# JuanDuGit/DH3D

Hardware: AMD Instinct MI355X
Metric: point-clouds/sec (higher is better)
Workload: dtype f32; 1 GPU; local-descriptor forward (basic_config), N=8192 K=8, batch=8; clouds_per_gpu=8, clouds_total=8, points=8192, knn=8, parallelism=clouds sharded over 1 GPU(s), no data-path collective, weights=random-init (no checkpoint blobs exist upstream), steps_in_flight=4

## Files before the change

dh3d_amd/csrc/knn.hip:

```cpp
#include <float.h>
#include <limits.h>

#include <type_traits>

#include "cell_walk.h"
#include "common.h"
#include "group_box.h"
#include "keys.h"
#include "wave_ops.h"

#pragma clang fp contract(off)

namespace {

typedef float f32x2 __attribute__((ext_vector_type(2)));
typedef unsigned long long u64;

constexpr int kQueriesPerBlock = 256;
constexpr int kChunk = 1024;
constexpr int kQueue = 16;

struct KnnLadder {
  int log2ct;
  int ctmask;
// ... 548 lines not shown
#pragma unroll
  for (int c = 0; c < CPL; ++c) kd[c] = ln + 64 * c < N ? __float_as_uint(sqrtf(s[c])) : 0xFFFFFFFFu;
  u64 need = 0;
  u64 m1 = ~0ull, m2 = ~0ull;
  bool more = false;
  auto rescan = [&]() {
    m1 = ~0ull; m2 = ~0ull;
    int cnt = 0;
    asm volatile("" : "+v"(ln));
#pragma unroll
    for (int c = 0; c < CPL; ++c) {
      const int j = ln + 64 * c;
      const unsigned tb = j < N ? (unsigned)((j & lad.ctmask) * lad.cv + (j >> lad.log2ct)) : 0xFFFFFFFFu;
      const u64 key = ((u64)kd[c] << 32) | tb;
      const bool ok = key >= need && key != ~0ull;
      const bool c1 = ok && key < m1, c2 = ok && key < m2;
      m2 = c1 ? m1 : (c2 ? key : m2);
      m1 = c1 ? key : m1;
      cnt += ok ? 1 : 0;
    }
    more = cnt > 2;
  };
  rescan();
  for (int r = 0; r < K; ++r) {
    const unsigned hi = wave_min_u32((unsigned)(m1 >> 32));
    const unsigned lo = wave_min_u32((unsigned)(m1 >> 32) == hi ? (unsigned)m1 : 0xFFFFFFFFu);
    if (lane == r) { my_hi = hi; my_lo = lo; }
    const u64 sel = ((u64)hi << 32) | lo;
    if (sel == ~0ull) break;
    need = sel + 1;
    const bool won = m1 == sel;
    const bool dry = won && m2 == ~0ull && more;
    m1 = won ? m2 : m1;
    m2 = won ? ~0ull : m2;
    if (__ballot(dry) != 0ull) rescan();
  }
}

template <int CPL, bool XYZ>
__global__ __launch_bounds__(256) void knn_small_kernel(const float *__restrict__ pos, int N, int K, KnnLadder lad,
                                                       int32_t *__restrict__ nn, float *__restrict__ dist, int Q) {
  __shared__ uint2 s_strip[4][64];
  const int b = blockIdx.y, lane = threadIdx.x & 63;
  const int wave = __builtin_amdgcn_readfirstlane(threadIdx.x >> 6);
  const int q0 = (blockIdx.x * 4 + wave) * Q;
  if (q0 >= N) return;
  const float *base = pos + (size_t)b * N * 3;
  float cx[CPL], cy[CPL], cz[CPL];
#pragma unroll
  for (int c = 0; c < CPL; ++c) {
    const int j = lane + 64 * c, jj = j < N ? j : 0;
    const float x = XYZ ? base[(size_t)jj * 3] : base[jj];
    cx[c] = j < N ? x : __builtin_nanf("");
    cy[c] = XYZ ? base[(size_t)jj * 3 + 1] : base[(size_t)N + jj];
    cz[c] = XYZ ? base[(size_t)jj * 3 + 2] : base[(size_t)2 * N + jj];
  }
  uint2 *strip = s_strip[wave];
#pragma unroll 1
  for (int qi = 0; qi < Q; ++qi) {
    const int q = q0 + qi;
    if (q >= N) break;
    const float qx = XYZ ? base[(size_t)q * 3] : base[q];
    const float qy = XYZ ? base[(size_t)q * 3 + 1] : base[(size_t)N + q];
    const float qz = XYZ ? base[(size_t)q * 3 + 2] : base[(size_t)2 * N + q];
    float s[CPL];
    float smin = __builtin_inff();
#pragma unroll
    for (int c = 0; c < CPL; ++c) {
      const float dx = qx - cx[c], dy = qy - cy[c], dz = qz - cz[c];
      s[c] = __builtin_fmaf(dz, dz, __builtin_fmaf(dy, dy, dx * dx));
      smin = fminf(smin, s[c]);
    }
    unsigned my_hi = 0xFFFFFFFFu, my_lo = 0xFFFFFFFFu;
    bool screened = K <= 8;
    int cnt = 0;
    if (screened) {
      const float ub = __fmul_rn(wave_max_of_min8_f32(smin), 1.000001f);
      int ln = lane;
      asm volatile("" : "+v"(ln));
#pragma unroll
      for (int c = 0; c < CPL; ++c) {
        const bool in = s[c] <= ub;
        const u64 mk = __ballot(in);
        const int at0 = cnt;
        cnt += __popcll(mk);
        if (in && cnt <= 64) {
          const unsigned at = __builtin_amdgcn_mbcnt_hi((unsigned)(mk >> 32), __builtin_amdgcn_mbcnt_lo((unsigned)mk, 0u));
          (strip + at0)[at] = make_uint2(__float_as_uint(s[c]), (unsigned)(ln + 64 * c));
        }
      }
      screened = cnt <= 64 && (cnt >= K || cnt >= N);
    }
    if (screened) {
      __builtin_amdgcn_fence(__ATOMIC_RELEASE, "wavefront");
      __builtin_amdgcn_wave_barrier();
      __builtin_amdgcn_fence(__ATOMIC_ACQUIRE, "wavefront");
      const uint2 e = strip[lane];
      const float d = sqrtf(__uint_as_float(e.x));
      const int j = (int)e.y;
      unsigned khi = lane < cnt ? __float_as_uint(d) : 0xFFFFFFFFu;
      unsigned klo = lane < cnt ? (unsigned)((j & lad.ctmask) * lad.cv + (j >> lad.log2ct)) : 0xFFFFFFFFu;
      for (int r = 0; r < K; ++r) {
        const unsigned hi = wave_min_u32(khi);
        const unsigned lo = wave_min_u32(khi == hi ? klo : 0xFFFFFFFFu);
        if (lane == r) { my_hi = hi; my_lo = lo; }
        if ((hi & lo) == 0xFFFFFFFFu) break;
        const bool won = khi == hi && klo == lo;
        khi = won ? 0xFFFFFFFFu : khi;
        klo = won ? 0xFFFFFFFFu : klo;
      }
      __builtin_amdgcn_fence(__ATOMIC_RELEASE, "wavefront");
    } else {
      knn_small_select_all<CPL>(s, N, K, lad, lane, my_hi, my_lo);
    }
    if (lane < K) {
      const size_t o = ((size_t)b * N + q) * K + lane;
      knn_emit(((u64)my_hi << 32) | my_lo, lad, nn + o, dist + o);
    }
  }
}

constexpr int kKnnMaxK = 64, kKnnMaxB = 65535;

static int knn_list_width(int K) { return K <= 4 ? 4 : K <= 8 ? 8 : K <= 16 ? 16 : K <= 32 ? 32 : 64; }

struct KnnPlan {
  int cpl, q, kmax;
};
static KnnPlan knn_plan(int B, int N, int K) {
  KnnPlan p{0, 0, 0};
  if (N <= 2048) {
    p.cpl = N <= 512 ? 8 : N <= 1024 ? 16 : 32;
    p.q = (long long)B * N <= 16384 ? 2 : 4;
    return p;
  }
  p.kmax = knn_list_width(K);
  return p;
}

constexpr int kAnyDpMax = 16;
static int knn_anydp_width(int K) { return K <= 8 ? 8 : K <= 16 ? 16 : 64; }

template <bool XYZ>
int knn_launch(const float *pos, int B, int N, int K, int32_t *nn, float *dist, hipStream_t s) {
  const KnnLadder lad = knn_ladder(N);
  const KnnPlan p = knn_plan(B, N, K);
  if (p.cpl > 0) {
    dim3 sgrid(dh3d_cdiv(N, 4 * p.q), B), sblock(256);
#define DH3D_SMALL_CASE(CPL)                                                                                     \
  if (p.cpl == CPL) {                                                                                            \
    hipLaunchKernelGGL((knn_small_kernel<CPL, XYZ>), sgrid, sblock, 0, s, pos, N, K, lad, nn, dist, p.q);        \
    return dh3d_launch_status();                                                                                 \
  }
    DH3D_SMALL_CASE(8) DH3D_SMALL_CASE(16) DH3D_SMALL_CASE(32)
#undef DH3D_SMALL_CASE
    return DH3D_ERR_UNSUPPORTED;
  }
  dim3 grid(dh3d_cdiv(N, kQueriesPerBlock), B), block(kQueriesPerBlock);
#define DH3D_LANE_CASE(KM)                                                                                       \
  if (p.kmax == KM) {                                                                                            \
    hipLaunchKernelGGL((knn_kernel<KM, XYZ>), grid, block, 0, s, pos, N, K, lad, nn, dist);                      \
    return dh3d_launch_status();                                                                                 \
  }
  DH3D_LANE_CASE(4) DH3D_LANE_CASE(8) DH3D_LANE_CASE(16) DH3D_LANE_CASE(32) DH3D_LANE_CASE(64)
#undef DH3D_LANE_CASE
  return DH3D_ERR_UNSUPPORTED;
}

template <int KMAX>
__global__ __launch_bounds__(256) void knn_anydp_kernel(const float *__restrict__ pos, int Dp, int N, int K, KnnLadder lad,
                                                        int32_t *__restrict__ nn, float *__restrict__ dist) {
  __shared__ float s_c[16][256];
  const int b = blockIdx.y, y = blockIdx.x * 256 + threadIdx.x;
  const float *pc = pos + (size_t)b * Dp * N;
  float q[16];
#pragma unroll
  for (int dp = 0; dp < 16; ++dp) q[dp] = (dp < Dp && y < N) ? pc[(size_t)dp * N + y] : 0.f;
  u64 keys[KMAX];
#pragma unroll
  for (int i = 0; i < KMAX; ++i) keys[i] = kKnnNoKey;
  for (int x0 = 0; x0 < N; x0 += 256) {
    __syncthreads();
    for (int dp = 0; dp < Dp; ++dp) s_c[dp][threadIdx.x] = x0 + (int)threadIdx.x < N ? pc[(size_t)dp * N + x0 + threadIdx.x] : 0.f;
    __syncthreads();
    const int cnt = min(256, N - x0);
    for (int j = 0; j < cnt; ++j) {
      float sum = 0.f;
      for (int dp = 0; dp < Dp; ++dp) {
        const float val = s_c[dp][j] - q[dp];
        sum = __builtin_fmaf(val, val, sum);
      }
      const float d = sqrtf(sum);
      const int x = x0 + j;
      const unsigned tb = (unsigned)((x & lad.ctmask) * lad.cv + (x >> lad.log2ct));
      const u64 key = ((u64)__float_as_uint(d) << 32) | tb;
      if (key < keys[K - 1]) {
        int i = K - 1;
        while (i > 0 && keys[i - 1] > key) { keys[i] = keys[i - 1]; --i; }
        keys[i] = key;
      }
    }
  }
  if (y >= N) return;
  int32_t *o_nn = nn + ((size_t)b * N + y) * K;
  float *o_d = dist + ((size_t)b * N + y) * K;
  for (int i = 0; i < K; ++i) knn_emit(keys[i], lad, o_nn + i, o_d + i);
}

}

DH3D_API int dh3d_knn_bruteforce(const float *positions, int B, int Dp, int N, int K, int32_t *nn,
                                 float *dist, void *stream) {
  DH3D_REQUIRE(positions && nn && dist && B > 0 && N > 0 && K > 0 && Dp > 0);
  DH3D_SUPPORTED(K <= kKnnMaxK && B <= kKnnMaxB);
  if (Dp == 3) return knn_launch<false>(positions, B, N, K, nn, dist, (hipStream_t)stream);
  DH3D_SUPPORTED(Dp <= kAnyDpMax);
  const KnnLadder lad = knn_ladder(N);
  dim3 grid(dh3d_cdiv(N, 256), B), block(256);
  hipStream_t s = (hipStream_t)stream;
  const int km = knn_anydp_width(K);
#define DH3D_ANYDP_CASE(KM)                                                                                      \
  if (km == KM) {                                                                                                \
    hipLaunchKernelGGL(knn_anydp_kernel<KM>, grid, block, 0, s, positions, Dp, N, K, lad, nn, dist);             \
    return dh3d_launch_status();                                                                                 \
  }
  DH3D_ANYDP_CASE(8) DH3D_ANYDP_CASE(16) DH3D_ANYDP_CASE(64)
#undef DH3D_ANYDP_CASE
  return DH3D_ERR_UNSUPPORTED;
}

DH3D_API int dh3d_knn_bruteforce_xyz(const float *xyz, int B, int N, int K, int32_t *nn, float *dist,
                                     void *stream) {
  DH3D_REQUIRE(xyz && nn && dist && B > 0 && N > 0 && K > 0);
  DH3D_SUPPORTED(K <= kKnnMaxK && B <= kKnnMaxB);
  return knn_launch<true>(xyz, B, N, K, nn, dist, (hipStream_t)stream);
}

DH3D_API int dh3d_knn_bruteforce_plan(int B, int Dp, int N, int K) {
  if (!(B > 0 && N > 0 && K > 0 && Dp > 0) || !(K <= kKnnMaxK && B <= kKnnMaxB)) return -1;
  if (Dp != 3) return Dp <= kAnyDpMax ? 3 * 65536 + knn_anydp_width(K) : -1;
  const KnnPlan p = knn_plan(B, N, K);
  return p.cpl > 0 ? 1 * 65536 + p.cpl * 256 + p.q : 2 * 65536 + p.kmax;
}

struct KnnSortedPlan {
  int s, kmax;
};
static KnnSortedPlan knn_sorted_plan(int B, int N, int K) {
  const long long groups = (long long)((N + 63) / 64) * B;
  KnnSortedPlan p{groups <= 256 ? 8 : groups <= 1280 ? 4 : groups <= 4096 ? 2 : 0, knn_list_width(K)};
  if (p.kmax > 16) p.s = 0;
  if (p.s == 8 && p.kmax == 4) p.kmax = 8;
  return p;
}

static int knn_sorted_launch(const float *sorted, const float *gbox, int B, int N, int K, int32_t *nn, float *dist,
                             const int *gate, void *stream) {
  DH3D_REQUIRE(sorted && gbox && nn && dist && B > 0 && N > 0 && K > 0);
  DH3D_SUPPORTED(K <= kKnnMaxK && B <= kKnnMaxB);
  const KnnLadder lad = knn_ladder(N);
  const int NG = (N + 63) / 64;
  dim3 grid(dh3d_cdiv(NG, kSortedWaves), B), block(64 * kSortedWaves);
  hipStream_t s = (hipStream_t)stream;
  const float4 *so = reinterpret_cast<const float4 *>(sorted);
  const KnnSortedPlan p = knn_sorted_plan(B, N, K);
  if (p.s > 0) {
    dim3 sgrid(NG, B);
#define DH3D_SPLIT_CASE(KM, SS)                                                                               \
  if (p.kmax == KM && p.s == SS) {                                                                           \
    hipLaunchKernelGGL((knn_split_kernel<KM, SS>), sgrid, dim3(64 * SS), 0, s, so, gbox, N, K, lad, nn, dist, gate); \
    return dh3d_launch_status();                                                                             \
  }
    DH3D_SPLIT_CASE(4, 2) DH3D_SPLIT_CASE(4, 4)
    DH3D_SPLIT_CASE(8, 2) DH3D_SPLIT_CASE(8, 4) DH3D_SPLIT_CASE(8, 8)
    DH3D_SPLIT_CASE(16, 2) DH3D_SPLIT_CASE(16, 4) DH3D_SPLIT_CASE(16, 8)
#undef DH3D_SPLIT_CASE
    return DH3D_ERR_UNSUPPORTED;
  }
#define DH3D_SORTED_CASE(KM)                                                                                  \
  if (p.kmax == KM) {                                                                                        \
    hipLaunchKernelGGL((knn_sorted_kernel<KM>), grid, block, 0, s, so, gbox, N, K, lad, nn, dist, gate);      \
    return dh3d_launch_status();                                                                             \
  }
  DH3D_SORTED_CASE(4) DH3D_SORTED_CASE(8) DH3D_SORTED_CASE(16) DH3D_SORTED_CASE(32) DH3D_SORTED_CASE(64)
#undef DH3D_SORTED_CASE
  return DH3D_ERR_UNSUPPORTED;
}

DH3D_API int dh3d_knn_sorted(const float *sorted, const float *gbox, int B, int N, int K, int32_t *nn,
                             float *dist, void *stream) {
  return knn_sorted_launch(sorted, gbox, B, N, K, nn, dist, nullptr, stream);
}

DH3D_API int dh3d_knn_sorted_plan(int B, int N, int K) {
  if (!(B > 0 && N > 0 && K > 0) || !(K <= kKnnMaxK && B <= kKnnMaxB)) return -1;
  const KnnSortedPlan p = knn_sorted_plan(B, N, K);
  return p.s * 256 + p.kmax;
}

constexpr int kGridCap = 256;
constexpr int kGridRow = kGridCap + 2;
constexpr int kGridScreenCap = 80;
static_assert(kGridScreenCap % 16 == 0 && kGridScreenCap * 6 <= kGridCap * 2, "the screened drain's row");

__device__ __forceinline__ unsigned knn_spread4(unsigned v) {
  return (v & 1u) | ((v & 2u) << 2) | ((v & 4u) << 4) | ((v & 8u) << 6);
}
__device__ __forceinline__ void knn_cswap(u64 &a, u64 &b) {
  const bool lt = b < a;
  const u64 lo = lt ? b : a, hi = lt ? a : b;
  a = lo; b = hi;
}
template <int CTRL>
__device__ __forceinline__ u64 knn_dpp_u64(u64 v) {
  const int lo = __builtin_amdgcn_update_dpp(0, (int)(unsigned)v, CTRL, 0xF, 0xF, true);
  const int hi = __builtin_amdgcn_update_dpp(0, (int)(unsigned)(v >> 32), CTRL, 0xF, 0xF, true);
  return ((u64)(unsigned)hi << 32) | (unsigned)lo;
}
template <int CTRL>
__device__ __forceinline__ int knn_dpp_i32(int v) {
  return __builtin_amdgcn_update_dpp(0, v, CTRL, 0xF, 0xF, true);
}
template <int CTRL>
__device__ __forceinline__ void knn_merge_step(KnnState<8> &st) {
  u64 c[8];
#pragma unroll
  for (int i = 0; i < 8; ++i) {
    const u64 mine = st.keys[i], theirs = knn_dpp_u64<CTRL>(st.keys[7 - i]);
    c[i] = mine < theirs ? mine : theirs;
  }
  knn_cswap(c[0], c[4]); knn_cswap(c[1], c[5]); knn_cswap(c[2], c[6]); knn_cswap(c[3], c[7]);
  knn_cswap(c[0], c[2]); knn_cswap(c[1], c[3]); knn_cswap(c[4], c[6]); knn_cswap(c[5], c[7]);
  knn_cswap(c[0], c[1]); knn_cswap(c[2], c[3]); knn_cswap(c[4], c[5]); knn_cswap(c[6], c[7]);
#pragma unroll
  for (int i = 0; i < 8; ++i) st.keys[i] = c[i];
}
__device__ __forceinline__ void knn_bound_of_list(KnnState<8> &st) {
  knn_inflated_sq((unsigned)(st.keys[7] >> 32), st.bound);
}
template <int L>
__device__ __forceinline__ void knn_merge_sublanes(KnnState<8> &st) {
  if (L >= 2) knn_merge_step<0xB1>(st);
  if (L >= 4) knn_merge_step<0x4E>(st);
  if (L >= 8) knn_merge_step<0x141>(st);
  knn_bound_of_list(st);
}
template <int L>
__device__ __forceinline__ void knn_merge_after_sparse_pass(KnnState<8> &st, int sub) {
  if (L != 4 || __any(sub != 0 && st.keys[0] != kKnnNoKey)) {
    knn_merge_sublanes<L>(st);
    return;
  }
#pragma unroll
  for (int i = 0; i < 8; ++i) st.keys[i] = knn_dpp_u64<0x00>(st.keys[i]);
  knn_bound_of_list(st);
}

template <int L, int SF>
__global__ __launch_bounds__(256) void knn_grid_kernel(const float4 *__restrict__ sorted, const float *__restrict__ gbox,
                                                      const int *__restrict__ cells, int N, int K, int D, KnnLadder lad,
                                                      int32_t *__restrict__ nn, float *__restrict__ dist) {
  constexpr int QB = 256 / L;
  static_assert(SF == 0 || (L == 4 && SF <= 4), "the merged scan: 64 queries per workgroup, at most four waves");
  constexpr int kGridLds = 3 * 64 * 4 + QB * kGridRow * 2 + QB * 4;
  constexpr int kSplitLds = SF == 2 ? 2 * knn_split_lds_bytes<2>() : SF > 0 ? knn_split_lds_bytes<(SF > 0 ? SF : 1)>() : 0;
  __shared__ __attribute__((aligned(16))) unsigned char s_raw[kGridLds > kSplitLds ? kGridLds : kSplitLds];
  const int b = blockIdx.y, lane = threadIdx.x & 63, sub = lane & (L - 1);
  if (cells[(size_t)b * kCellInts + kCellFlag]) {
    if constexpr (SF > 0) {
      const int ngq = (N + 63) / 64;
      if constexpr (SF == 2) {
        const int half = (int)(threadIdx.x >> 7), pairs = (ngq + 1) / 2;
        if ((int)blockIdx.x >= pairs) return;
        const int g0 = (int)blockIdx.x + half * pairs;
        if (g0 >= ngq) return;
        knn_split_body<8, 2>(sorted, gbox, N, K, lad, nn, dist, b, (int)(((unsigned)g0 + 37u * (unsigned)b) % (unsigned)ngq),
                             s_raw + half * knn_split_lds_bytes<2>(), half * 2);
      } else if (threadIdx.x < 64 * SF) {
        knn_split_body<8, (SF > 0 ? SF : 1)>(sorted, gbox, N, K, lad, nn, dist, b, (int)((blockIdx.x + 37u * (unsigned)b) % (unsigned)ngq), s_raw);
      }
    }
    return;
  }
  const int qi = (int)((blockIdx.x + 37u * (unsigned)b) % gridDim.x) * QB + threadIdx.x / L;
  const bool valid = qi < N;
  const float4 *sc = sorted + (size_t)b * N;
  const CellGrid g = cell_grid(cells, b);
  const int *ct = g.ct;
  const float lo[3] = {g.lo[0], g.lo[1], g.lo[2]}, scl[3] = {g.scl[0], g.scl[1], g.scl[2]};
  const int nb[3] = {g.nb[0], g.nb[1], g.nb[2]};
  const float4 qr = sc[valid ? qi : N - 1];
  const float q[3] = {qr.x, qr.y, qr.z};
  int nc[3], drop[3];
  sched_bits(g.sched, nc, kGridSteps - D);
#pragma unroll
  for (int a = 0; a < 3; ++a) drop[a] = nb[a] - nc[a];
  const int span = 1 << D;
  int cq[3], gmax[3];
  float w[3], eps[3];
#pragma unroll
  for (int a = 0; a < 3; ++a) {
    cq[a] = min((4 << nb[a]) - 1, max(0, (int)((q[a] - lo[a]) * scl[a]))) >> (2 + drop[a]);
    gmax[a] = ((1 << nb[a]) >> drop[a]) - 1;
    w[a] = (float)(4 << drop[a]) / scl[a];
    eps[a] = 2.5e-6f * ((float)(4 << nb[a]) / scl[a]);
  }
  unsigned (*s_ctab)[64] = reinterpret_cast<unsigned (*)[64]>(s_raw);
  cell_deposit_tables(g.sched, nc[0], nc[1], nc[2], kGridSteps - D, s_ctab);
  auto tab_code = [&](int ax, int ay, int az) { return s_ctab[0][ax & 63] | s_ctab[1][ay & 63] | s_ctab[2][az & 63]; };
  KnnState<8> st;
  knn_list_reset(st);
  if (!valid) st.bound = -1.f;

  auto axis_d2 = [&](int a, int o) {
    const float l = lo[a] + (float)(cq[a] + o) * w[a];
    const float d = fmaxf(fmaxf(fmaxf(l - q[a], q[a] - (l + w[a])), 0.f) - eps[a], 0.f);
    return d * d;
  };
  float d2x[5];
  unsigned bitx[5];
  bool okx[5];
#pragma unroll
  for (int t = 0; t < 5; ++t) {
    const int ax = cq[0] + t - 2;
    okx[t] = (unsigned)ax <= (unsigned)gmax[0];
    d2x[t] = okx[t] ? axis_d2(0, t - 2) : INFINITY;
    bitx[t] = s_ctab[0][ax & 63];
  }
  auto inside = [&](int R) {
    float G = INFINITY;
#pragma unroll
    for (int a = 0; a < 3; ++a) {
      if (cq[a] - R > 0) G = fminf(G, (q[a] - (lo[a] + (float)(cq[a] - R) * w[a])) - eps[a]);
      if (cq[a] + R < gmax[a]) G = fminf(G, ((lo[a] + (float)(cq[a] + R + 1) * w[a]) - q[a]) - eps[a]);
    }
    if (G == INFINITY) return true;
    G = fmaxf(G, 0.f);
    return st.bound < G * G * 0.99999f;
  };

  auto keep_one_copy = [&]() {
    if (sub != 0) knn_list_clear(st);
  };
  unsigned short (*s_list)[kGridRow] = reinterpret_cast<unsigned short (*)[kGridRow]>(s_raw + 3 * 64 * 4);
  int *s_cnt = reinterpret_cast<int *>(s_raw + 3 * 64 * 4 + QB * kGridRow * 2);
  const int qs = threadIdx.x / L;
  auto direct = [&](int j) {
    const float4 r = sc[j];
    const float dx = r.x - q[0], dy = r.y - q[1], dz = r.z - q[2];
    knn_offer<8, false>(st, fmaf(dz, dz, fmaf(dy, dy, dx * dx)), __float_as_int(r.w), lad);
  };
  auto enqueue = [&](int beg, int end) {
    const int len = end - beg;
    if (len <= 0) return;
    const int off = atomicAdd(&s_cnt[qs], len);
    const int fit = min(len, kGridCap - off);
    for (int k = 0; k < fit; ++k) s_list[qs][off + k] = (unsigned short)(beg + k);
    for (int k = max(fit, 0); k < len; ++k) direct(beg + k);
  };
  auto drain_screened = [&]() __attribute__((always_inline)) {
    const int T = s_cnt[qs];
    if constexpr (L != 4) return min(T, kGridCap);
    const bool screen = !__any(T > kGridScreenCap) && __any(T > 32);
    const int ns = screen ? T : 0;
    unsigned short *row = s_list[qs];
    float *s2v = reinterpret_cast<float *>(row + kGridScreenCap);
    float m1 = INFINITY, m2 = INFINITY;
#pragma unroll 1
    for (int k0 = 0; k0 < ns; k0 += 4 * L) {
      float4 r[4];
#pragma unroll
      for (int u = 0; u < 4; ++u) r[u] = sc[row[min(k0 + sub + u * L, ns - 1)]];
      wave_lds_sync();
#pragma unroll
      for (int u = 0; u < 4; ++u) {
        const int i = k0 + sub + u * L;
        const float dx = r[u].x - q[0], dy = r[u].y - q[1], dz = r[u].z - q[2];
        const float s = i < ns ? fmaf(dz, dz, fmaf(dy, dy, dx * dx)) : __builtin_nanf("");
        m2 = s < m1 ? m1 : fminf(m2, s);
        m1 = fminf(m1, s);
        s2v[i] = s;
        row[i] = (unsigned short)__float_as_int(r[u].w);
      }
    }
    float U = m2;
    U = fmaxf(U, __int_as_float(knn_dpp_i32<0xB1>(__float_as_int(U))));
    U = fmaxf(U, __int_as_float(knn_dpp_i32<0x4E>(__float_as_int(U))));
    const float thr = __fmul_rn(U, 1.000001f);
    wave_lds_sync();
    int c = 0;
#pragma unroll 1
    for (int k0 = 0; k0 < ns; k0 += 4 * L) {
      float s[4];
      unsigned short id[4];
#pragma unroll
      for (int u = 0; u < 4; ++u) {
        s[u] = s2v[k0 + sub + u * L];
        id[u] = row[k0 + sub + u * L];
      }
      wave_lds_sync();
      int n = 0, at[4];
#pragma unroll
      for (int u = 0; u < 4; ++u) {
        at[u] = n;
        n += s[u] <= thr ? 1 : 0;
      }
      const int n1 = knn_dpp_i32<0x90>(n);
      int p = n + (sub >= 1 ? n1 : 0);
      const int p2 = knn_dpp_i32<0x40>(p);
      p += sub >= 2 ? p2 : 0;
      const int first = c + p - n;
#pragma unroll
      for (int u = 0; u < 4; ++u)
        if (s[u] <= thr) {
          s2v[first + at[u]] = s[u];
          row[first + at[u]] = id[u];
        }
      c += knn_dpp_i32<0xFF>(p);
      wave_lds_sync();
    }
    float s_n = s2v[sub];
    int id_n = row[sub];
#pragma unroll 1
    for (int j = sub; j < c; j += L) {
      const float s = s_n;
      const int id = id_n;
      const int jn = min(j + L, kGridScreenCap - 1);
      s_n = s2v[jn];
      id_n = row[jn];
      knn_offer<8, false>(st, s, id, lad);
    }
    return screen ? 0 : min(T, kGridCap);
  };
  auto drain = [&](auto screen) __attribute__((always_inline)) {
    wave_lds_sync();
    int total;
    if constexpr (decltype(screen)::value) total = drain_screened();
    else total = min(s_cnt[qs], kGridCap);
#pragma unroll 1
    for (int base = sub; base < total; base += 4 * L) {
      float4 r[4];
      bool ok[4];
#pragma unroll
      for (int u = 0; u < 4; ++u) {
        const int i = base + u * L;
        ok[u] = i < total;
        r[u] = sc[s_list[qs][min(i, total - 1)]];
      }
#pragma unroll
      for (int u = 0; u < 4; ++u) {
        const float dx = r[u].x - q[0], dy = r[u].y - q[1], dz = r[u].z - q[2];
        const float s2 = fmaf(dz, dz, fmaf(dy, dy, dx * dx));
        knn_offer<8, false>(st, ok[u] ? s2 : __builtin_nanf(""), __float_as_int(r[u].w), lad);
      }
    }
    wave_lds_sync();
  };
  auto column = [&](auto tmask, int dy, int dz) __attribute__((always_inline)) {
    constexpr int TMASK = decltype(tmask)::value;
    const int ay = cq[1] + dy - 2, az = cq[2] + dz - 2;
    if ((unsigned)ay > (unsigned)gmax[1] || (unsigned)az > (unsigned)gmax[2]) return;
    const float d2yz = axis_d2(1, dy - 2) + axis_d2(2, dz - 2);
    const unsigned bityz = tab_code(0, ay, az);
    int beg[5], end[5];
#pragma unroll
    for (int t = 0; t < 5; ++t)
      if (TMASK >> t & 1) {
        beg[t] = ct[bityz | bitx[t]];
        end[t] = ct[(bityz | bitx[t]) + span];
      }
    if constexpr (TMASK != 0b01110) {
#pragma unroll
      for (int t = 0; t < 5; ++t)
        if (TMASK >> t & 1) {
          if (!okx[t] || (d2yz + d2x[t]) * 0.99999f > st.bound) continue;
          enqueue(beg[t], end[t]);
        }
    } else {
      int len[5], tot = 0;
#pragma unroll
      for (int t = 0; t < 5; ++t)
        if (TMASK >> t & 1) {
          len[t] = okx[t] && !((d2yz + d2x[t]) * 0.99999f > st.bound) ? end[t] - beg[t] : 0;
          tot += len[t];
        }
      if (tot == 0) return;
      int off = atomicAdd(&s_cnt[qs], tot);
#pragma unroll
      for (int t = 0; t < 5; ++t)
        if (TMASK >> t & 1) {
          const int fit = min(len[t], kGridCap - off);
          unsigned short *dst = &s_list[qs][off];
#pragma unroll
          for (int k = 0; k < 4; ++k)
            if (k < fit) dst[k] = (unsigned short)(beg[t] + k);
          for (int k = 4; k < fit; ++k) dst[k] = (unsigned short)(beg[t] + k);
          for (int k = max(fit, 0); k < len[t]; ++k) direct(beg[t] + k);
          off += len[t];
        }
    }
  };
  auto begin_pass = [&]() __attribute__((always_inline)) {
    if (sub == 0) s_cnt[qs] = 0;
    __builtin_amdgcn_fence(__ATOMIC_SEQ_CST, "wavefront");
    __builtin_amdgcn_wave_barrier();
  };
  begin_pass();
  if constexpr (L == 4) {
    const int ay = cq[1] + 1, az = cq[2] + 1;
    const bool mine = sub < 3 && (unsigned)ay <= (unsigned)gmax[1] && (unsigned)az <= (unsigned)gmax[2];
    const bool okc = sub == 0 ? okx[1] : sub == 1 ? okx[2] : okx[3];
    const float d2c = (sub == 0 ? d2x[1] : sub == 1 ? d2x[2] : d2x[3]) + axis_d2(1, 1) + axis_d2(2, 1);
    const unsigned code = tab_code(0, ay, az) | (sub == 0 ? bitx[1] : sub == 1 ? bitx[2] : bitx[3]);
    const int beg9 = ct[mine ? code : 0], end9 = ct[mine ? code + span : 0];
#pragma unroll 1
    for (int ci = sub; ci < 8; ci += L) column(std::integral_constant<int, 0b01110>{}, 1 + ci % 3, 1 + ci / 3);
    if (mine && okc && !(d2c * 0.99999f > st.bound)) enqueue(beg9, end9);
  } else {
#pragma unroll 1
    for (int ci = sub; ci < 9; ci += L) column(std::integral_constant<int, 0b01110>{}, 1 + ci % 3, 1 + ci / 3);
  }
  drain(std::true_type{});
  knn_merge_sublanes<L>(st);
  keep_one_copy();
  begin_pass();
  bool exact = false;
  int ylo = -2, zlo = -2, ny = 5, ncol = valid ? 25 : 0;
  if (valid && st.bound < INFINITY) {
    const float r = sqrtf(st.bound) * 1.0001f;
    int dlo[3], dhi[3];
#pragma unroll
    for (int a = 0; a < 3; ++a) {
      const float inv = scl[a] / (float)(4 << drop[a]);
      dlo[a] = min(0, max(0, (int)floorf((q[a] - r - eps[a] - lo[a]) * inv)) - cq[a]);
      dhi[a] = max(0, min(gmax[a], (int)floorf((q[a] + r + eps[a] - lo[a]) * inv)) - cq[a]);
    }
    const int by = dhi[1] - dlo[1] + 1, bc = by * (dhi[2] - dlo[2] + 1);
    if (dlo[0] >= -2 && dhi[0] <= 2 && bc <= 128) {
      exact = true;
      ylo = dlo[1]; zlo = dlo[2]; ny = by; ncol = bc;
    }
  }
#pragma unroll 1
  for (int ci = sub; ci < ncol; ci += L) {
    const int iz = ci / ny, dy = ylo + (ci - iz * ny), dz = zlo + iz;
    if (abs(dy) <= 1 && abs(dz) <= 1) column(std::integral_constant<int, 0b10001>{}, dy + 2, dz + 2);
    else column(std::integral_constant<int, 0b11111>{}, dy + 2, dz + 2);
  }
  drain(std::false_type{});
  knn_merge_after_sparse_pass<L>(st, sub);
  const bool done = !valid || exact || inside(2);
  if (__any(!done)) {
    if (done) {
      keep_one_copy();
    } else {
      knn_list_clear(st);
      const int NG = (N + 63) >> 6;
      const float4 *gb = reinterpret_cast<const float4 *>(gbox) + (size_t)b * NG * 2;
#pragma unroll 1
      for (int g = sub; g < NG; g += L) {
        const float4 lo4 = gb[2 * g], hi4 = gb[2 * g + 1];
        if (point_box_gap2(lo4, hi4, q[0], q[1], q[2]) > st.bound) continue;
        const int j1 = min(N, g * 64 + 64);
#pragma unroll 1
        for (int j = g * 64; j < j1; j += 8) {
          float4 r8[8];
#pragma unroll
          for (int u = 0; u < 8; ++u) r8[u] = sc[min(j + u, j1 - 1)];
#pragma unroll
          for (int u = 0; u < 8; ++u) {
            const float dx = r8[u].x - q[0], dy = r8[u].y - q[1], dz = r8[u].z - q[2];
            const float s2 = fmaf(dz, dz, fmaf(dy, dy, dx * dx));
            knn_offer<8, false>(st, j + u < j1 ? s2 : __builtin_nanf(""), __float_as_int(r8[u].w), lad);
          }
        }
      }
    }
    knn_merge_sublanes<L>(st);
  }
  if (valid) {
    const int y = __float_as_int(qr.w);
#pragma unroll
    for (int e = 0; e < 8 / L; ++e) {
      const int slot = e * L + sub;
      if (slot >= K) break;
      u64 key = st.keys[0];
#pragma unroll
      for (int i = 1; i < 8; ++i) key = slot == i ? st.keys[i] : key;
      const size_t o = ((size_t)b * N + y) * K + slot;
      knn_emit(key, lad, nn + o, dist + o);
    }
  }
}

constexpr int kGridLanes = 4;

struct KnnGridPlan {
  int sf, drop;
};
static KnnGridPlan knn_grid_plan(int B, int N) {
  KnnGridPlan p{0, 0};
  while (p.drop < 6 && ((long long)N << p.drop) <= 3072) ++p.drop;
  const long long groups = (long long)((N + 63) / 64) * B;
  if (kGridLanes == 4 && groups <= 4096) p.sf = groups > 1280 ? 2 : 4;
  return p;
}

DH3D_API int dh3d_knn_grid_plan(int B, int N, int K) {
  if (B <= 0 || N <= 0 || K <= 0 || K > 8 || N > 16384 || B > 65535) return -1;
  const KnnGridPlan p = knn_grid_plan(B, N);
  return p.sf + 16 * p.drop;
}

DH3D_API int dh3d_knn_grid(const float *sorted, const float *gbox, const int32_t *cells, int B, int N, int K, int32_t *nn,
                           float *dist, void *stream) {
  DH3D_REQUIRE(sorted && gbox && cells && nn && dist && B > 0 && N > 0 && K > 0);
  DH3D_SUPPORTED(K <= 8 && N <= 16384 && B <= 65535);
  const KnnLadder lad = knn_ladder(N);
  constexpr int kLanes = kGridLanes;
  const KnnGridPlan plan = knn_grid_plan(B, N);
  const int D = plan.drop;
  const dim3 grid(dh3d_cdiv(N, 256 / kLanes), B);
  const float4 *so = reinterpret_cast<const float4 *>(sorted);
  if (plan.sf == 2) {
    hipLaunchKernelGGL((knn_grid_kernel<4, 2>), grid, dim3(256), 0, (hipStream_t)stream, so, gbox, cells, N, K, D, lad, nn, dist);
    return dh3d_launch_status();
  }
  if (plan.sf == 4) {
    hipLaunchKernelGGL((knn_grid_kernel<4, 4>), grid, dim3(256), 0, (hipStream_t)stream, so, gbox, cells, N, K, D, lad, nn, dist);
    return dh3d_launch_status();
  }
  hipLaunchKernelGGL((knn_grid_kernel<kLanes, 0>), grid, dim3(256), 0, (hipStream_t)stream, so, gbox, cells, N, K, D, lad, nn, dist);
  if (dh3d_launch_status() != DH3D_OK) return DH3D_ERR_LAUNCH;
  return knn_sorted_launch(sorted, gbox, B, N, K, nn, dist, cells, stream);
}
```

Before: 41330 point-clouds/sec.

## Pool second-pass shell cells across the wave instead of per-query column loops

The second grid pass used to walk up to 25 columns of five cells for each query on its own sub-lanes. It now computes each query's exact bounding box shell beyond the 3x3x3 core, prefix-sums the shell cell counts across the wave, and stores per-query records in LDS. Every lane then takes one cell from the pooled wave-wide list, culls it against that query's bound, and appends its points to the query's list. This is meant to balance uneven per-query cell work across lanes and to drop the fixed 5x5 column scan. In exchange it adds LDS records, binary searches and integer-division tricks, and it adds a new fallback to brute force when a list overflows or the box is wide.

```diff
diff --git a/dh3d_amd/csrc/knn.hip b/dh3d_amd/csrc/knn.hip
--- a/dh3d_amd/csrc/knn.hip
+++ b/dh3d_amd/csrc/knn.hip
@@ -874,6 +874,41 @@
 constexpr int kGridRow = kGridCap + 2;
 constexpr int kGridScreenCap = 80;
 static_assert(kGridScreenCap % 16 == 0 && kGridScreenCap * 6 <= kGridCap * 2, "the screened drain's row");
+constexpr int kGridBoxCells = 640;
+
+struct alignas(16) KnnBoxRec {
+  float4 qb;
+  int4 box;
+};
+__device__ __forceinline__ int knn_pack3(int x, int y, int z) { return x | (y << 8) | (z << 16); }
+__device__ __forceinline__ int knn_byte(int v, int a) { return (v >> (8 * a)) & 0xFF; }
+
+static_assert(2.125 * kGridBoxCells * kGridBoxCells < (1 << 20), "knn_small_div");
+__device__ __forceinline__ int knn_small_div(int t, int d) {
+  const unsigned m = (unsigned)(1048576.f * __builtin_amdgcn_rcpf((float)d)) + 2u;
+  return (int)(((unsigned)t * m) >> 20);
+}
+
+__device__ __forceinline__ int knn_box_shell(int lo0, int lo1, int lo2, int hi0, int hi1, int hi2, int t, int &dx, int &dy, int &dz) {
+  const int in00 = max(lo0, -1), in01 = max(lo1, -1), in02 = max(lo2, -1);
+  const int in10 = min(hi0, 1), in11 = min(hi1, 1), in12 = min(hi2, 1);
+  const int b0 = hi0 - lo0 + 1, b1 = hi1 - lo1 + 1, b2 = hi2 - lo2 + 1;
+  const int i0 = in10 - in00 + 1, i1 = in11 - in01 + 1, i2 = in12 - in02 + 1;
+  const int nz = b0 * b1 * (b2 - i2), ny = b0 * i2 * (b1 - i1), nx = i1 * i2 * (b0 - i0);
+  const int g = t < nz ? 0 : t < nz + ny ? 1 : 2;
+  t -= g == 0 ? 0 : g == 1 ? nz : nz + ny;
+  const int d1 = g == 2 ? i1 : b0, d2 = g == 0 ? b1 : i2;
+  const int u = knn_small_div(t, d1), f = t - u * d1;
+  const int k = knn_small_div(u, d2), s = u - k * d2;
+  const int slo = g == 0 ? lo2 : g == 1 ? lo1 : lo0;
+  const int sin0 = g == 0 ? in02 : g == 1 ? in01 : in00;
+  const int sin1 = g == 0 ? in12 : g == 1 ? in11 : in10;
+  const int v = k < sin0 - slo ? slo + k : sin1 + 1 + (k - (sin0 - slo));
+  dx = g == 2 ? v : lo0 + f;
+  dy = g == 2 ? in01 + f : g == 1 ? v : lo1 + s;
+  dz = g == 0 ? v : in02 + s;
+  return nz + ny + nx;
+}
 
 __device__ __forceinline__ unsigned knn_spread4(unsigned v) {
   return (v & 1u) | ((v & 2u) << 2) | ((v & 4u) << 4) | ((v & 8u) << 6);
@@ -934,7 +969,10 @@
                                                       int32_t *__restrict__ nn, float *__restrict__ dist) {
   constexpr int QB = 256 / L;
   static_assert(SF == 0 || (L == 4 && SF <= 4), "the merged scan: 64 queries per workgroup, at most four waves");
-  constexpr int kGridLds = 3 * 64 * 4 + QB * kGridRow * 2 + QB * 4;
+  constexpr int QW = 64 / L;
+  constexpr int kGridRecAt = 3 * 64 * 4 + QB * kGridRow * 2 + QB * 4;
+  constexpr int kGridLds = kGridRecAt + QB * (int)sizeof(KnnBoxRec);
+  static_assert(kGridRecAt % 16 == 0 && (L != 4 || kGridLds <= 40 * 1024), "16-byte records; four workgroups per CU");
   constexpr int kSplitLds = SF == 2 ? 2 * knn_split_lds_bytes<2>() : SF > 0 ? knn_split_lds_bytes<(SF > 0 ? SF : 1)>() : 0;
   __shared__ __attribute__((aligned(16))) unsigned char s_raw[kGridLds > kSplitLds ? kGridLds : kSplitLds];
   const int b = blockIdx.y, lane = threadIdx.x & 63, sub = lane & (L - 1);
@@ -984,19 +1022,20 @@
   knn_list_reset(st);
   if (!valid) st.bound = -1.f;
 
-  auto axis_d2 = [&](int a, int o) {
-    const float l = lo[a] + (float)(cq[a] + o) * w[a];
-    const float d = fmaxf(fmaxf(fmaxf(l - q[a], q[a] - (l + w[a])), 0.f) - eps[a], 0.f);
+  auto cell_d2 = [&](int a, float qa, int c) __attribute__((always_inline)) {
+    const float l = lo[a] + (float)c * w[a];
+    const float d = fmaxf(fmaxf(fmaxf(l - qa, qa - (l + w[a])), 0.f) - eps[a], 0.f);
     return d * d;
   };
-  float d2x[5];
-  unsigned bitx[5];
-  bool okx[5];
-#pragma unroll
-  for (int t = 0; t < 5; ++t) {
-    const int ax = cq[0] + t - 2;
+  auto axis_d2 = [&](int a, int o) __attribute__((always_inline)) { return cell_d2(a, q[a], cq[a] + o); };
+  float d2x[3];
+  unsigned bitx[3];
+  bool okx[3];
+#pragma unroll
+  for (int t = 0; t < 3; ++t) {
+    const int ax = cq[0] + t - 1;
     okx[t] = (unsigned)ax <= (unsigned)gmax[0];
-    d2x[t] = okx[t] ? axis_d2(0, t - 2) : INFINITY;
+    d2x[t] = okx[t] ? axis_d2(0, t - 1) : INFINITY;
     bitx[t] = s_ctab[0][ax & 63];
   }
   auto inside = [&](int R) {
@@ -1128,48 +1167,35 @@
     }
     wave_lds_sync();
   };
-  auto column = [&](auto tmask, int dy, int dz) __attribute__((always_inline)) {
-    constexpr int TMASK = decltype(tmask)::value;
-    const int ay = cq[1] + dy - 2, az = cq[2] + dz - 2;
+  auto column = [&](int dy, int dz) __attribute__((always_inline)) {
+    const int ay = cq[1] + dy, az = cq[2] + dz;
     if ((unsigned)ay > (unsigned)gmax[1] || (unsigned)az > (unsigned)gmax[2]) return;
-    const float d2yz = axis_d2(1, dy - 2) + axis_d2(2, dz - 2);
+    const float d2yz = axis_d2(1, dy) + axis_d2(2, dz);
     const unsigned bityz = tab_code(0, ay, az);
-    int beg[5], end[5];
-#pragma unroll
-    for (int t = 0; t < 5; ++t)
-      if (TMASK >> t & 1) {
-        beg[t] = ct[bityz | bitx[t]];
-        end[t] = ct[(bityz | bitx[t]) + span];
-      }
-    if constexpr (TMASK != 0b01110) {
-#pragma unroll
-      for (int t = 0; t < 5; ++t)
-        if (TMASK >> t & 1) {
-          if (!okx[t] || (d2yz + d2x[t]) * 0.99999f > st.bound) continue;
-          enqueue(beg[t], end[t]);
-        }
-    } else {
-      int len[5], tot = 0;
-#pragma unroll
-      for (int t = 0; t < 5; ++t)
-        if (TMASK >> t & 1) {
-          len[t] = okx[t] && !((d2yz + d2x[t]) * 0.99999f > st.bound) ? end[t] - beg[t] : 0;
-          tot += len[t];
-        }
-      if (tot == 0) return;
-      int off = atomicAdd(&s_cnt[qs], tot);
-#pragma unroll
-      for (int t = 0; t < 5; ++t)
-        if (TMASK >> t & 1) {
-          const int fit = min(len[t], kGridCap - off);
-          unsigned short *dst = &s_list[qs][off];
-#pragma unroll
-          for (int k = 0; k < 4; ++k)
-            if (k < fit) dst[k] = (unsigned short)(beg[t] + k);
-          for (int k = 4; k < fit; ++k) dst[k] = (unsigned short)(beg[t] + k);
-          for (int k = max(fit, 0); k < len[t]; ++k) direct(beg[t] + k);
-          off += len[t];
-        }
+    int beg[3], end[3];
+#pragma unroll
+    for (int t = 0; t < 3; ++t) {
+      beg[t] = ct[bityz | bitx[t]];
+      end[t] = ct[(bityz | bitx[t]) + span];
+    }
+    int len[3], tot = 0;
+#pragma unroll
+    for (int t = 0; t < 3; ++t) {
+      len[t] = okx[t] && !((d2yz + d2x[t]) * 0.99999f > st.bound) ? end[t] - beg[t] : 0;
+      tot += len[t];
+    }
+    if (tot == 0) return;
+    int off = atomicAdd(&s_cnt[qs], tot);
+#pragma unroll
+    for (int t = 0; t < 3; ++t) {
+      const int fit = min(len[t], kGridCap - off);
+      unsigned short *dst = &s_list[qs][off];
+#pragma unroll
+      for (int k = 0; k < 4; ++k)
+        if (k < fit) dst[k] = (unsigned short)(beg[t] + k);
+      for (int k = 4; k < fit; ++k) dst[k] = (unsigned short)(beg[t] + k);
+      for (int k = max(fit, 0); k < len[t]; ++k) direct(beg[t] + k);
+      off += len[t];
     }
   };
   auto begin_pass = [&]() __attribute__((always_inline)) {
@@ -1181,47 +1207,92 @@
   if constexpr (L == 4) {
     const int ay = cq[1] + 1, az = cq[2] + 1;
     const bool mine = sub < 3 && (unsigned)ay <= (unsigned)gmax[1] && (unsigned)az <= (unsigned)gmax[2];
-    const bool okc = sub == 0 ? okx[1] : sub == 1 ? okx[2] : okx[3];
-    const float d2c = (sub == 0 ? d2x[1] : sub == 1 ? d2x[2] : d2x[3]) + axis_d2(1, 1) + axis_d2(2, 1);
-    const unsigned code = tab_code(0, ay, az) | (sub == 0 ? bitx[1] : sub == 1 ? bitx[2] : bitx[3]);
+    const bool okc = sub == 0 ? okx[0] : sub == 1 ? okx[1] : okx[2];
+    const float d2c = (sub == 0 ? d2x[0] : sub == 1 ? d2x[1] : d2x[2]) + axis_d2(1, 1) + axis_d2(2, 1);
+    const unsigned code = tab_code(0, ay, az) | (sub == 0 ? bitx[0] : sub == 1 ? bitx[1] : bitx[2]);
     const int beg9 = ct[mine ? code : 0], end9 = ct[mine ? code + span : 0];
 #pragma unroll 1
-    for (int ci = sub; ci < 8; ci += L) column(std::integral_constant<int, 0b01110>{}, 1 + ci % 3, 1 + ci / 3);
+    for (int ci = sub; ci < 8; ci += L) column(ci % 3 - 1, ci / 3 - 1);
     if (mine && okc && !(d2c * 0.99999f > st.bound)) enqueue(beg9, end9);
   } else {
 #pragma unroll 1
-    for (int ci = sub; ci < 9; ci += L) column(std::integral_constant<int, 0b01110>{}, 1 + ci % 3, 1 + ci / 3);
+    for (int ci = sub; ci < 9; ci += L) column(ci % 3 - 1, ci / 3 - 1);
   }
   drain(std::true_type{});
   knn_merge_sublanes<L>(st);
-  keep_one_copy();
-  begin_pass();
-  bool exact = false;
-  int ylo = -2, zlo = -2, ny = 5, ncol = valid ? 25 : 0;
+  bool exact = false, wide = false;
+  int blo[3] = {0, 0, 0}, bhi[3] = {0, 0, 0};
   if (valid && st.bound < INFINITY) {
     const float r = sqrtf(st.bound) * 1.0001f;
-    int dlo[3], dhi[3];
 #pragma unroll
     for (int a = 0; a < 3; ++a) {
       const float inv = scl[a] / (float)(4 << drop[a]);
-      dlo[a] = min(0, max(0, (int)floorf((q[a] - r - eps[a] - lo[a]) * inv)) - cq[a]);
-      dhi[a] = max(0, min(gmax[a], (int)floorf((q[a] + r + eps[a] - lo[a]) * inv)) - cq[a]);
-    }
-    const int by = dhi[1] - dlo[1] + 1, bc = by * (dhi[2] - dlo[2] + 1);
-    if (dlo[0] >= -2 && dhi[0] <= 2 && bc <= 128) {
-      exact = true;
-      ylo = dlo[1]; zlo = dlo[2]; ny = by; ncol = bc;
-    }
-  }
+      blo[a] = min(0, max(0, (int)floorf((q[a] - r - eps[a] - lo[a]) * inv)) - cq[a]);
+      bhi[a] = max(0, min(gmax[a], (int)floorf((q[a] + r + eps[a] - lo[a]) * inv)) - cq[a]);
+    }
+    wide = (bhi[0] - blo[0] + 1) * (bhi[1] - blo[1] + 1) * (bhi[2] - blo[2] + 1) > kGridBoxCells;
+    exact = !wide;
+  } else if (valid) {
+#pragma unroll
+    for (int a = 0; a < 3; ++a) {
+      blo[a] = max(-2, -cq[a]);
+      bhi[a] = min(2, gmax[a] - cq[a]);
+    }
+  }
+  int ncell, unused[3];
+  ncell = knn_box_shell(blo[0], blo[1], blo[2], bhi[0], bhi[1], bhi[2], 0, unused[0], unused[1], unused[2]);
+  if (wide) ncell = 0;
+  int last = ncell;
+#pragma unroll
+  for (int off = L; off < 64; off <<= 1) {
+    const int o = __shfl_up(last, off, 64);
+    if (lane >= off) last += o;
+  }
+  const int wave_cells = __builtin_amdgcn_readlane(last, 63);
+  bool full = false;
+  if (wave_cells > 0) {
+    KnnBoxRec *s_rec = reinterpret_cast<KnnBoxRec *>(s_raw + kGridRecAt);
+    const int q0 = qs & ~(QW - 1);
+    if (sub == 0) {
+      s_cnt[qs] = 0;
+      s_rec[qs].qb = make_float4(q[0], q[1], q[2], st.bound);
+      s_rec[qs].box = make_int4(knn_pack3(cq[0], cq[1], cq[2]), knn_pack3(-blo[0], -blo[1], -blo[2]),
+                                knn_pack3(bhi[0], bhi[1], bhi[2]), last - ncell);
+    }
+    wave_lds_sync();
+    bool pooled = false;
 #pragma unroll 1
-  for (int ci = sub; ci < ncol; ci += L) {
-    const int iz = ci / ny, dy = ylo + (ci - iz * ny), dz = zlo + iz;
-    if (abs(dy) <= 1 && abs(dz) <= 1) column(std::integral_constant<int, 0b10001>{}, dy + 2, dz + 2);
-    else column(std::integral_constant<int, 0b11111>{}, dy + 2, dz + 2);
-  }
-  drain(std::false_type{});
-  knn_merge_after_sparse_pass<L>(st, sub);
-  const bool done = !valid || exact || inside(2);
+    for (int base = 0; base < wave_cells; base += 64) {
+      const int j = base + lane;
+      if (j >= wave_cells) continue;
+      int f = 0;
+#pragma unroll
+      for (int step = QW / 2; step > 0; step >>= 1)
+        if (s_rec[q0 + f + step].box.w <= j) f += step;
+      const float4 fq = s_rec[q0 + f].qb;
+      const int4 fb = s_rec[q0 + f].box;
+      int fd[3], fc[3];
+      knn_box_shell(-knn_byte(fb.y, 0), -knn_byte(fb.y, 1), -knn_byte(fb.y, 2), knn_byte(fb.z, 0), knn_byte(fb.z, 1),
+                    knn_byte(fb.z, 2), j - fb.w, fd[0], fd[1], fd[2]);
+#pragma unroll
+      for (int a = 0; a < 3; ++a) fc[a] = knn_byte(fb.x, a) + fd[a];
+      const unsigned code = tab_code(fc[0], fc[1], fc[2]);
+      const int beg = ct[code], len = ct[code + span] - beg;
+      const float d2 = (cell_d2(1, fq.y, fc[1]) + cell_d2(2, fq.z, fc[2])) + cell_d2(0, fq.x, fc[0]);
+      if (d2 * 0.99999f > fq.w || len <= 0) continue;
+      pooled = true;
+      const int off = atomicAdd(&s_cnt[q0 + f], len);
+      const int fit = min(len, kGridCap - off);
+      for (int k = 0; k < fit; ++k) s_list[q0 + f][off + k] = (unsigned short)(beg + k);
+    }
+    if (__any(pooled)) {
+      keep_one_copy();
+      drain(std::false_type{});
+      knn_merge_after_sparse_pass<L>(st, sub);
+      full = s_cnt[qs] > kGridCap;
+    }
+  }
+  const bool done = !valid || (!full && !wide && (exact || inside(2)));
   if (__any(!done)) {
     if (done) {
       keep_one_copy();
```

New measurement: 41890 point-clouds/sec, median of 6. 1.01x the previous value.
